# Dyllon-Preston/trajopt-grpo

Hardware: AMD Instinct MI355X
Metric: env-steps/sec at 65k parallel quadrotor envs (rollout + PPO update) (higher is better)
Workload: dtype bf16 (f32 accumulate) MLP; f32 env / returns / loss / optimizer

## Files before the change

### include/trajopt_grpo_hip.h

```cpp
#ifndef TRAJOPT_GRPO_HIP_H
#define TRAJOPT_GRPO_HIP_H

#include <stdint.h>

#ifdef __cplusplus
extern "C" {
#endif

#define TG_ABI_VERSION 13

enum { TG_OK = 0, TG_ERR_ARG = -1, TG_ERR_HIP = -2, TG_ERR_UNSUPPORTED = -3 };

#define TG_ACT_RELU 0
#define TG_ACT_TANH 1

enum { TG_ENV_CARTPOLE = 0, TG_ENV_QUADPOLE2D = 1, TG_ENV_QUADPOLE = 2, TG_ENV_QUADROTOR12 = 3, TG_ENV_PENDULUM = 4 };
enum { TG_F32 = 0, TG_F64 = 1 };

typedef struct tg_env_params {
    int32_t env_id;
    int32_t max_steps;
    int32_t time_trunc_step;
    int32_t agents;
    double  timestep;
    double  p[12];
} tg_env_params;

typedef struct tg_traj {
    void*     d_obs;
    float*    d_act;
    void*     d_rew;
    uint8_t*  d_mask;
    int32_t*  d_len;
    uint64_t* d_counters;
    int64_t   n;
    int32_t   horizon;
    int32_t   dtype;
} tg_traj;

const char* tg_last_error(void);
int  tg_abi_version(void);
int  tg_chain_depth_kernels(int on);

int  tg_env_dims(int env_id, int* obs_dim, int* act_dim);
int  tg_env_default_params(int env_id, int max_steps, tg_env_params* out);
int  tg_env_finalize_params(tg_env_params* p);

int  tg_env_reset(const tg_env_params* p, int dtype, void* d_state, int64_t ld, int64_t n,
                  uint64_t seed, uint64_t stream_id, int64_t key_offset, int64_t key_div,
                  void* stream);

int  tg_env_step(const tg_env_params* p, int dtype, const void* d_state, int64_t ld,
                 const float* d_action, int64_t ld_a, void* d_next, int64_t ld_next,
                 int32_t* d_steps, void* d_time_balanced, void* d_reward,
                 uint8_t* d_truncated, int64_t n, void* stream);

int  tg_quadrotor12_dynamics(const tg_env_params* p, int dtype, const void* d_state, int64_t ld,
                             const void* d_control, int64_t ld_c, void* d_next, int64_t ld_next,
                             int64_t n, void* stream);


int  tg_rollout_begin(const tg_traj* tr, int obs_dim, int act_dim, void* stream);

int  tg_rollout_step(const tg_env_params* p, const tg_traj* tr, int32_t t, const float* d_mean,
                     int64_t mean_row_stride, const float* sigma, const uint64_t* d_rng,
// ... 499 lines not shown
```

### trajopt-grpo_amd/_native.py

```python
from __future__ import annotations

import ctypes as C
import os

import torch

_HERE = os.path.dirname(os.path.abspath(__file__))
LIB_PATH = os.environ.get("TG_NATIVE_LIB") or os.path.join(_HERE, "libtrajopt_grpo_hip.so")
ABI_VERSION = 13

TG_ENV_CARTPOLE, TG_ENV_QUADPOLE2D, TG_ENV_QUADPOLE, TG_ENV_QUADROTOR12, TG_ENV_PENDULUM = 0, 1, 2, 3, 4
TG_F32, TG_F64 = 0, 1
TG_OK, TG_ERR_ARG, TG_ERR_HIP, TG_ERR_UNSUPPORTED = 0, -1, -2, -3
TG_ACT_RELU, TG_ACT_TANH = 0, 1
ENV_IDS = {"CartPole": TG_ENV_CARTPOLE, "QuadPole2D": TG_ENV_QUADPOLE2D, "QuadPole": TG_ENV_QUADPOLE,
           "Quadrotor": TG_ENV_QUADROTOR12, "Pendulum": TG_ENV_PENDULUM}


class NativeLibraryError(RuntimeError):
    pass


class EnvParams(C.Structure):
    _fields_ = [("env_id", C.c_int32), ("max_steps", C.c_int32), ("time_trunc_step", C.c_int32),
# ... 92 lines not shown
                ("d_act_rows", C.c_void_p), ("d_idx", C.c_void_p), ("d_src0", C.c_void_p), ("d_dst0", C.c_void_p),
                ("d_src1", C.c_void_p), ("d_dst1", C.c_void_p), ("d_moments", C.c_void_p), ("group_size", C.c_int64),
                ("rows_cap", C.c_int64)]


class VecEnv(C.Structure):
    _fields_ = [("d_state", C.c_void_p), ("d_steps", C.c_void_p), ("d_balanced", C.c_void_p), ("d_ep_return", C.c_void_p),
                ("d_episode", C.c_void_p), ("n", C.c_int64), ("env_offset", C.c_int64), ("seed", C.c_uint64), ("horizon", C.c_int32),
                ("dtype", C.c_int32)]


class Replay(C.Structure):
    _fields_ = [("d_obs", C.c_void_p), ("d_act", C.c_void_p), ("d_next_obs", C.c_void_p), ("d_rew", C.c_void_p), ("d_disc", C.c_void_p),
                ("d_nstep", C.c_void_p), ("d_last_obs", C.c_void_p), ("d_cursor", C.c_void_p), ("d_filled", C.c_void_p),
                ("d_open", C.c_void_p), ("n", C.c_int64), ("capacity_steps", C.c_int32), ("obs_dim", C.c_int32), ("act_dim", C.c_int32),
                ("n_step", C.c_int32), ("discount", C.c_float * 17)]


_P, _I32, _I64, _U64, _F, _VP = C.POINTER, C.c_int32, C.c_int64, C.c_uint64, C.c_float, C.c_void_p
SIGNATURES = {
    "tg_last_error": (C.c_char_p, []),
    "tg_abi_version": (C.c_int, []),
    "tg_chain_depth_kernels": (C.c_int, [C.c_int]),
    "tg_env_dims": (C.c_int, [C.c_int, _P(C.c_int), _P(C.c_int)]),
    "tg_env_default_params": (C.c_int, [C.c_int, C.c_int, _P(EnvParams)]),
    "tg_env_finalize_params": (C.c_int, [_P(EnvParams)]),
    "tg_env_reset": (C.c_int, [_P(EnvParams), C.c_int, _VP, _I64, _I64, _U64, _U64, _I64, _I64, _VP]),
    "tg_env_step": (C.c_int, [_P(EnvParams), C.c_int, _VP, _I64, _VP, _I64, _VP, _I64, _VP, _VP, _VP, _VP, _I64, _VP]),
    "tg_quadrotor12_dynamics": (C.c_int, [_P(EnvParams), C.c_int, _VP, _I64, _VP, _I64, _VP, _I64, _I64, _VP]),
    "tg_rollout_begin": (C.c_int, [_P(Traj), C.c_int, C.c_int, _VP]),
    "tg_rollout_step": (C.c_int, [_P(EnvParams), _P(Traj), _I32, _VP, _I64, _P(_F), _VP, _I64, _VP]),
    "tg_rollout_forced": (C.c_int, [_P(EnvParams), _P(Traj), _I32, _I32, _VP]),
    "tg_rollout_final_state": (C.c_int, [_P(EnvParams), _P(Traj), _VP, _VP, _VP]),
    "tg_rollout_finish": (C.c_int, [_P(Traj), _VP]),
    "tg_rollout_finish_stats_workspace": (C.c_int, []),
    "tg_rollout_finish_stats": (C.c_int, [_P(Traj), _VP, _VP, _VP, _VP]),
    "tg_fused_rollout": (C.c_int, [_P(EnvParams), _P(Traj), _VP, _VP, _I32, _I32, _P(_F), _VP, _I64, _I32, _I32, _VP]),
    "tg_fused_rollout_f32_supported": (C.c_int, [_I32, _I32]),
    "tg_fused_rollout_f32_block_envs": (C.c_int, [_I64, _I32]),
    "tg_fused_rollout_f32": (C.c_int, [_P(EnvParams), _P(Traj), _VP, _VP, _I32, _I32, _I32, _P(_F), _VP, _I64, _I32, _I32, _VP]),
    "tg_fused_rollout_f32_act": (C.c_int, [_P(EnvParams), _P(Traj), _VP, _VP, _I32, _I32, _I32, _P(_F), _VP, _I64, _I32, _I32, _I32, _VP]),
    "tg_rng_advance": (C.c_int, [_VP, _VP]),
    "tg_env_randomize": (C.c_int, [_P(EnvParams), _P(RandomizeSpec), _VP, _I64, _U64, _U64, _I64, _I64, _VP]),
    "tg_rollout_step_dr": (C.c_int, [_P(EnvParams), _VP, _P(Traj), _I32, _VP, _I64, _P(_F), _VP, _I64, _VP]),
    "tg_rollout_forced_dr": (C.c_int, [_P(EnvParams), _VP, _P(Traj), _I32, _I32, _VP]),
    "tg_rollout_final_state_dr": (C.c_int, [_P(EnvParams), _VP, _P(Traj), _VP, _VP, _VP]),
# ... 193 lines not shown
        raise RuntimeError(f"{what or 'trajopt_grpo_hip'} failed ({rc}): {msg}")


def require_cuda(*tensors):
    for t in tensors:
        if t is not None and not t.is_cuda:
            raise NativeLibraryError("the HIP rollout path needs tensors on an MI355X (cuda) device; got a CPU tensor. "
                                     "There is no CPU fallback.")


def ptr(t):
    return 0 if t is None else t.data_ptr()


RAW_PARAM_WRITES = [0]
ALWAYS_REBUILD = os.environ.get("TG_ALWAYS_REBUILD", "0") == "1"
TRUST_KEYS = os.environ.get("TG_TRUST_VERSION_KEYS", "0") == "1"


def chain_depth_kernels_default():
    return os.environ.get("TG_CHAIN_DEPTH_KERNELS", "1") != "0"


def event_pair():
    return (torch.cuda.Event(enable_timing=True), torch.cuda.Event(enable_timing=True))


def stream_ptr(device=None):
    return torch.cuda.current_stream(device).cuda_stream


def dtype_code(dt):
    if dt == torch.float32:
        return TG_F32
    if dt == torch.float64:
        return TG_F64
    raise ValueError(f"state dtype must be float32 or float64, got {dt}")


def default_params(env_id, max_steps):
    p = EnvParams()
    check(load().tg_env_default_params(env_id, int(max_steps), C.byref(p)), "tg_env_default_params")
    return p


def env_dims(env_id):
# ... 4 lines not shown
```

### trajopt-grpo_amd/csrc/api_common.cpp

```cpp
#include "tg_common.hpp"
#include <atomic>

namespace tg {

static thread_local char g_err[512] = "";

int set_error(int code, const char* fmt, ...) {
    va_list ap;
    va_start(ap, fmt);
    vsnprintf(g_err, sizeof(g_err), fmt, ap);
    va_end(ap);
    return code;
}

static std::atomic<int> g_chain_depth_kernels{1};
bool chain_depth_kernels() { return g_chain_depth_kernels.load(std::memory_order_relaxed) != 0; }

}

extern "C" {
const char* tg_last_error(void) { return tg::g_err; }
int tg_abi_version(void) { return TG_ABI_VERSION; }
int tg_chain_depth_kernels(int on) { return tg::g_chain_depth_kernels.exchange(on != 0 ? 1 : 0, std::memory_order_relaxed); }

int tg_clock_probe_attach(int32_t family, void* d_probe) {
    switch (family) {
        case TG_PROBE_FWD_CHAIN: return tg::attach_probe_fwd_chain(d_probe);
        case TG_PROBE_BWD_CHAIN: return tg::attach_probe_bwd_chain(d_probe);
        case TG_PROBE_WEIGHT_GRAD: return tg::attach_probe_weight_grad(d_probe);
        case TG_PROBE_F32_CHAIN: { const int rc = tg::attach_probe_f32(0, d_probe); return rc ? rc : tg::attach_probe_f32w(0, d_probe); }
        case TG_PROBE_F32_WEIGHT_GRAD: { const int rc = tg::attach_probe_f32(1, d_probe); return rc ? rc : tg::attach_probe_f32w(1, d_probe); }
        case TG_PROBE_MFMA_LOOP: return tg::attach_probe_mfma_loop(d_probe);
        case TG_PROBE_FWD_CHAIN_PLAIN: return tg::attach_probe_fwd_chain_plain(d_probe);
        default: return tg::set_error(TG_ERR_ARG, "tg_clock_probe_attach: family %d", family);
    }
}
}
```

### trajopt-grpo_amd/csrc/mfma_ring.hpp

```cpp
#pragma once
#include "tg_common.hpp"

namespace tg {

typedef __bf16 bf16x8 __attribute__((ext_vector_type(8)));
typedef float f32x16 __attribute__((ext_vector_type(16)));
typedef float f32x4 __attribute__((ext_vector_type(4)));
typedef __attribute__((address_space(3))) void lds_void;

typedef unsigned int act_u32x4 __attribute__((ext_vector_type(4)));
__device__ static inline void act_store16(act_u32x4 v, act_u32x4* p) {
    __builtin_nontemporal_store(v, p);
}

template <int H>
struct PanelOrder {
    static constexpr int CG = H / 32;
    static constexpr int ROWQ = CG * 256;
    static constexpr int PANEL = 8 * ROWQ;
    __host__ __device__ static constexpr int64_t chunk_off(int64_t row, int c) {
        return (row >> 5) * PANEL + ((row >> 2) & 7) * ROWQ + (c >> 2) * 256 + (row & 3) * 64 + (c & 3) * 16;
    }
    __host__ __device__ static constexpr int64_t store_row(int64_t row, int64_t rows) {
        return row < ((rows + 31) & ~(int64_t)31) ? row : rows - 1;
// ... 56 lines not shown
    CUR = ring + cur_slot * KS * 64;                                                                       \
    cur_slot = (cur_slot + 1 == D) ? 0 : cur_slot + 1;
#define TG_RING_NEXT    \
    const uint4* cur;   \
    TG_RING_NEXT_INTO(cur)
#define TG_RING_ADVANCE(WAITN) TG_RING_WAIT(WAITN) TG_RING_NEXT

template <int KS, int WPW, int D, int NB>
__device__ static inline const uint4* ring_next_at(const uint4*& wfrag, uint4* ring, int c, int wave, uint32_t& voff) {
    static_assert(NB % D == 0, "the ring must be back at slot 0 after every round");
    constexpr int P = D - 1;
    __builtin_amdgcn_s_barrier();
    asm volatile("" : "+v"(voff), "+s"(wfrag) : : "memory");
    const char* gblock = reinterpret_cast<const char*>(wfrag) + ((c + P) % NB) * (KS * 1024);
    uint4* slot = ring + ((c + P) % D) * (KS * 64);
#pragma unroll
    for (int q = 0; q < KS / WPW; ++q) {
        const int piece = q * WPW + wave;
        __builtin_amdgcn_global_load_lds(reinterpret_cast<const uint4*>(gblock + piece * 1024 + voff), (lds_void*)(slot + piece * 64), 16, 0, 0);
    }
    return ring + (c % D) * (KS * 64);
}

}
```

### trajopt-grpo_amd/csrc/mlp_fwd_chain.hip

```cpp
#include "mfma_ring.hpp"
#include "loss_row.hpp"

namespace tg {

typedef float f32x4 __attribute__((ext_vector_type(4)));

constexpr int kChainMaxHidden = 8;
TG_CLOCK_PROBE_VAR(g_probe_fwd_chain, attach_probe_fwd_chain)
TG_CLOCK_PROBE_VAR(g_probe_fwd_chain_plain, attach_probe_fwd_chain_plain)
struct ChainActs { uint16_t* p[kChainMaxHidden]; uint32_t* m[kChainMaxHidden]; };

struct ChainLoss {
    int32_t kind, A;
    const float* act;
    const float* logp_old; const float* adv;
    float n_m, n_i;
    float inv_var[4]; float logp_const, epsilon, surr_coef, critic_coef, kl_coef;
    const float* norm8;
    uint16_t* dout8;
    float* head_slabs;
    double* work;
    float* bias_partial;
    const float* logp_ref; float ref_coef;
    const float* log_std; float* std_out;
// ... 74 lines not shown
    f32x4 acc[2][2];
#pragma unroll
    for (int f = 0; f < 2; ++f) {
        const float4 b4 = lds_float4(b8 + 4 * f);
#pragma unroll
        for (int c = 0; c < 2; ++c) acc[f][c] = f32x4{b4.x, b4.y, b4.z, b4.w};
    }
    __builtin_amdgcn_s_setprio(1);
#pragma unroll
    for (int ks = 0; ks < K8; ++ks)
#pragma unroll
        for (int f = 0; f < 2; ++f) {
            const bf16x8 a = __builtin_bit_cast(bf16x8, cur[(ks * 2 + f) * 64 + lane]);
#pragma unroll
            for (int c = 0; c < 2; ++c) acc[f][c] = __builtin_amdgcn_mfma_f32_16x16x32_bf16(a, xin[c][ks], acc[f][c], 0, 0, 0);
        }
    __builtin_amdgcn_s_setprio(0);
#pragma unroll
    for (int c = 0; c < 2; ++c)
        out[c] = relu_pack_bf16(acc[0][c][0], acc[0][c][1], acc[0][c][2], acc[0][c][3], acc[1][c][0], acc[1][c][1], acc[1][c][2],
                                acc[1][c][3]);
}

__device__ static inline int wave_of(unsigned tid) { return (int)(tid >> 6); }

#define TG_CHAIN_ADVANCE(WAITN) TG_RING_ADVANCE(WAITN)

template <int H, int WPW, bool kStore, int D, bool kA0, bool kHead = false, bool kRef = false, bool kStd = false, bool kPanel = false>
__global__ __launch_bounds__(64 * WPW, 2) void mlp_fwd_chain_kernel(const uint16_t* __restrict__ x, const uint4* __restrict__ wfrag,
                                                                    const float* __restrict__ bias, int32_t n_hh, int64_t rows,
                                                                    ChainActs acts, float* __restrict__ out, int32_t out_cols,
                                                                    ChainLoss L) {
    static_assert(!kHead || (kStore && !kA0), "the fused head belongs to the learner's training pass");
    static_assert(!kRef || kHead, "the reference penalty is a term of the fused head");
    static_assert(!kStd || kHead, "the learned log-std is a term of the fused head");
    static_assert(!kPanel || (kStore && D == 4), "panel order is a layout of the stored activations; its wait counts are for P = 3");
    if constexpr (kHead) loss_from_device<kStd>(L);
    constexpr int MT = H / 32, KS = H / 16, K8 = H / 32;
    constexpr int P = D - 1;
    static_assert(P % 2 == 1 && P >= 3, "the store counts below are for a window of an odd number of blocks");
    constexpr int kWaitEven = (P - 1) * (KS / WPW) + (kStore ? 4 * ((P + 1) / 2) : 0);
    constexpr int kWaitOdd = (P - 1) * (KS / WPW) + (kStore ? 4 * ((P - 1) / 2) : 0);
    constexpr int kWaitMin = (P - 1) * (KS / WPW);
#define TG_PANEL_WAIT(S)                                                                    \
    if ((S) == 0) { TG_RING_WAIT(kWaitMin) } else if ((S) == 1) { TG_RING_WAIT(kWaitMin + 2) } \
    else if ((S) == 2) { TG_RING_WAIT(kWaitMin + 4) } else { TG_RING_WAIT(kWaitMin + 6) }
    static_assert(KS % WPW == 0, "every wave moves the same number of 1-KiB pieces per block");
    extern __shared__ uint4 lds[];
    uint4* ring = lds;
    float* bias_s = reinterpret_cast<float*>(lds + D * KS * 64);
    uint4* xs = reinterpret_cast<uint4*>(bias_s + (n_hh + 2) * H);
    uint4* stage = xs + WPW * 128 + wave_of(threadIdx.x) * (32 * 8);
#define TG_HEAD_LDS                                                                                                              \
    char* tiles = reinterpret_cast<char*>(xs + WPW * 128);                                                                       \
    char* dtiles = tiles + WPW * 32 * 128;                                                                                       \
    [[maybe_unused]] float* lin = reinterpret_cast<float*>(dtiles + WPW * 1024) + wave_of(threadIdx.x) * 256;                    \
    [[maybe_unused]] double* sums_d = reinterpret_cast<double*>(dtiles + 2 * WPW * 1024) + (wave_of(threadIdx.x) * 16 + (threadIdx.x & 15)) * 4; \
    [[maybe_unused]] float* sums_f = reinterpret_cast<float*>(dtiles + 2 * WPW * 1024 + WPW * 16 * 32) + (wave_of(threadIdx.x) * 16 + (threadIdx.x & 15)) * 4; \
    [[maybe_unused]] float* hacc = reinterpret_cast<float*>(dtiles + 2 * WPW * 1024 + WPW * 16 * 48) + (wave_of(threadIdx.x) * MT * 16 + (threadIdx.x & 15)) * 4;

    const int lane = threadIdx.x & 63, wave = threadIdx.x >> 6;
    const int grp = lane >> 4, col = lane & 15;
    const int64_t n_rounds = (rows + 32 * WPW - 1) / (32 * WPW);
    const int n_blocks = n_hh * MT + 2;
    if constexpr (kHead) { TG_CLOCK_PROBE_BEGIN(g_probe_fwd_chain) } else { TG_CLOCK_PROBE_BEGIN(g_probe_fwd_chain_plain) }

    for (int q = threadIdx.x; q < (n_hh + 2) * H; q += 64 * WPW) bias_s[q] = bias[q];
    if constexpr (kHead) {
        TG_HEAD_LDS
        if (grp == 0) {
#pragma unroll
            for (int b = 0; b < MT; ++b) *reinterpret_cast<float4*>(hacc + b * 64) = float4{0.f, 0.f, 0.f, 0.f};
            lds_stored2(sums_d, double2{0.0, 0.0});
            lds_stored2(sums_d + 2, double2{0.0, 0.0});
            *reinterpret_cast<float4*>(sums_f) = float4{0.f, 0.f, 0.f, 0.f};
        }
    }
    __syncthreads();

    uint4* my_xs = xs + wave * 128;
    auto dma_x = [&](int64_t round) {
        const int64_t base = round * (32 * WPW) + wave * 32;
#pragma unroll
        for (int p = 0; p < 2; ++p) {
// ... 10 lines not shown
            int64_t r = round * (32 * WPW) + wave * 32 + lane;
            r = r < rows ? r : rows - 1;
            if (L.kind != 1) {
#pragma unroll
                for (int k = 0; k < 4; ++k)
                    if (k < L.A) __builtin_amdgcn_global_load_lds(L.act + r * L.A + k, (lds_void*)(lin + 32 * k), 4, 0, 0);
                __builtin_amdgcn_global_load_lds(L.logp_old + r, (lds_void*)(lin + 32 * 4), 4, 0, 0);
                __builtin_amdgcn_global_load_lds(L.adv + r, (lds_void*)(lin + 32 * 5), 4, 0, 0);
                if constexpr (kRef) __builtin_amdgcn_global_load_lds(L.logp_ref + r, (lds_void*)(lin + 32 * 6), 4, 0, 0);
            } else {
                __builtin_amdgcn_global_load_lds(L.act + r, (lds_void*)(lin + 32 * 0), 4, 0, 0);
            }
        }
    };
    int pre_pos = 0, pre_slot = 0, cur_slot = 0;
    dma_x(blockIdx.x);
    if constexpr (kHead) dma_loss_inputs(blockIdx.x);
    for (int b0 = 0; b0 < P; ++b0) {
        ring_dma_block<KS, WPW>(wfrag + (int64_t)pre_pos * KS * 64, ring + pre_slot * KS * 64, wave, lane);
        pre_pos = (pre_pos + 1 == n_blocks) ? 0 : pre_pos + 1;
        pre_slot = (pre_slot + 1 == D) ? 0 : pre_slot + 1;
    }
    asm volatile("s_waitcnt vmcnt(0)" ::: "memory");

    for (int64_t round = blockIdx.x; round < n_rounds; round += gridDim.x) {
        const int64_t row0 = round * (32 * WPW) + wave * 32;
        int64_t rowc[2];
#pragma unroll
        for (int c = 0; c < 2; ++c) {
            rowc[c] = row0 + 16 * c + col;
            rowc[c] = rowc[c] < rows ? rowc[c] : rows - 1;
        }
        bf16x8 xin[2][K8], xout[2][K8];
        [[maybe_unused]] int64_t poff[2];
        if constexpr (kPanel) {
#pragma unroll
            for (int c = 0; c < 2; ++c) poff[c] = PanelOrder<H>::chunk_off(PanelOrder<H>::store_row(row0 + 16 * c + col, rows), grp);
        }

        {
            if constexpr (kHead) { TG_RING_WAIT(kWaitMin) } else { TG_RING_WAIT(kWaitOdd) }
            TG_RING_NEXT
            bf16x8 x0[2];
#pragma unroll
            for (int c = 0; c < 2; ++c) x0[c] = __builtin_bit_cast(bf16x8, lds_read_b128_opaque(my_xs + (16 * c + col) * 4 + grp));
            dma_x(round + gridDim.x);
#pragma unroll
            for (int mt = 0; mt < MT; ++mt) {
                f32x4 acc[2][2];
#pragma unroll
                for (int f = 0; f < 2; ++f) {
                    const float4 b4 = lds_float4(bias_s + 32 * mt + 8 * grp + 4 * f);
                    const bf16x8 a = __builtin_bit_cast(bf16x8, cur[(mt * 2 + f) * 64 + lane]);
#pragma unroll
                    for (int c = 0; c < 2; ++c)
                        acc[f][c] = __builtin_amdgcn_mfma_f32_16x16x32_bf16(a, x0[c], f32x4{b4.x, b4.y, b4.z, b4.w}, 0, 0, 0);
                }
#pragma unroll
                for (int c = 0; c < 2; ++c)
                    xout[c][mt] = relu_pack_bf16(acc[0][c][0], acc[0][c][1], acc[0][c][2], acc[0][c][3], acc[1][c][0], acc[1][c][1],
                                                 acc[1][c][2], acc[1][c][3]);
                if constexpr (kPanel) {
                    if (kA0) {
                        const bf16x8 pv[2] = {xout[0][mt], xout[1][mt]};
                        store_panel<H>(acts.p[0], poff, mt, pv);
                    }
                } else if (kStore && kA0 && (mt & 1)) {
                    const bf16x8 pa[2] = {xout[0][mt - 1], xout[1][mt - 1]}, pb[2] = {xout[0][mt], xout[1][mt]};
                    store_pair(stage, acts.p[0] + 32 * (mt - 1), row0, rows, H, lane, pa, pb);
                }
            }
#pragma unroll
            for (int c = 0; c < 2; ++c)
#pragma unroll
                for (int ks = 0; ks < K8; ++ks) xin[c][ks] = xout[c][ks];
        }
        for (int l = 0; l < n_hh; ++l) {
            const float* bl = bias_s + (l + 1) * H + 8 * grp;
            uint32_t mw[2][MT / 2];
#pragma unroll
            for (int mt = 0; mt < MT; ++mt) {
                const bool top_layer = kHead && l == n_hh - 1;
                if constexpr (kPanel) {
                    const int same = mt < 3 ? mt : 3;
                    if (top_layer) { TG_PANEL_WAIT(3 - same) } else if (l == 0) { TG_PANEL_WAIT(same) } else { TG_PANEL_WAIT(3) }
                } else if ((kStore && !kA0 && l == 0 && mt < 3) || (top_layer && mt >= 3)) {
                    TG_RING_WAIT(kWaitMin)
                } else if ((mt & 1) || (top_layer && mt == 2)) {
                    TG_RING_WAIT(kWaitOdd)
                } else {
                    TG_RING_WAIT(kWaitEven)
                }
                TG_RING_NEXT
                if (kStore) {
                    const int q = mt;
                    mw[q / (MT / 2)][q % (MT / 2)] = pair_mask_word(xin[q / (MT / 2)], q % (MT / 2), 4 * (grp & 1));
                }
                bf16x8 o[2];
                chain_block<K8>(cur, bl + 32 * mt, xin, o, lane);
                xout[0][mt] = o[0];
                xout[1][mt] = o[1];
                if constexpr (kPanel) {
                    if (mt == MT - 1 && acts.m[l]) {
#pragma unroll
                        for (int c = 0; c < 2; ++c) store_mask_words<MT>(acts.m[l], rowc[c], grp, mw[c]);
                    }
                    if (!top_layer) store_panel<H>(acts.p[l + 1], poff, mt, o);
                } else if (mt & 1) {
                    if (kStore && mt == MT - 1 && acts.m[l]) {
#pragma unroll
                        for (int c = 0; c < 2; ++c) store_mask_words<MT>(acts.m[l], rowc[c], grp, mw[c]);
                    }
                    if (kStore && !top_layer) {
                        const bf16x8 pa[2] = {xout[0][mt - 1], xout[1][mt - 1]}, pb[2] = {xout[0][mt], xout[1][mt]};
                        store_pair(stage, acts.p[l + 1] + 32 * (mt - 1), row0, rows, H, lane, pa, pb);
                    }
                }
            }
#pragma unroll
            for (int c = 0; c < 2; ++c)
#pragma unroll
                for (int ks = 0; ks < K8; ++ks) xin[c][ks] = xout[c][ks];
        }
        {
            if constexpr (kHead) { TG_RING_WAIT(kWaitMin) } else if constexpr (kPanel) { TG_PANEL_WAIT(3) } else { TG_RING_WAIT(kWaitEven) }
            TG_RING_NEXT
            if (kStore && acts.m[n_hh]) {
#pragma unroll
                for (int c = 0; c < 2; ++c) {
                    uint32_t mw[MT / 2];
#pragma unroll
                    for (int i = 0; i < MT / 2; ++i) mw[i] = pair_mask_word(xin[c], i, 4 * (grp & 1));
                    store_mask_words<MT>(acts.m[n_hh], rowc[c], grp, mw);
                }
            }
            const float4 b4 = lds_float4(bias_s + (n_hh + 1) * H + 4 * grp);
            f32x4 acc[2] = {f32x4{b4.x, b4.y, b4.z, b4.w}, f32x4{b4.x, b4.y, b4.z, b4.w}};
#pragma unroll
            for (int ks = 0; ks < K8; ++ks) {
                const bf16x8 a = __builtin_bit_cast(bf16x8, cur[(ks * 2) * 64 + lane]);
#pragma unroll
                for (int c = 0; c < 2; ++c) acc[c] = __builtin_amdgcn_mfma_f32_16x16x32_bf16(a, xin[c][ks], acc[c], 0, 0, 0);
            }
            if (out != nullptr && 4 * grp < out_cols) {
#pragma unroll
                for (int c = 0; c < 2; ++c)
                    *reinterpret_cast<float4*>(out + rowc[c] * out_cols + 4 * grp) = float4{acc[c][0], acc[c][1], acc[c][2], acc[c][3]};
            }
            if constexpr (kHead) {
                TG_HEAD_LDS
                char* dt = dtiles + wave * 1024;
                if (grp == 0) {
#pragma unroll 1
                    for (int c = 0; c < 2; ++c) {
                        float c_surr = 0.f, c_crit = 0.f, c_kl = 0.f, c_cnt = 0.f;
                        const int rl = 16 * c + col;
                        const bool valid = row0 + rl < rows;
                        float g[4] = {0.f, 0.f, 0.f, 0.f};
                        const f32x4 mu = c == 0 ? acc[0] : acc[1];
                        const int64_t rc = c == 0 ? rowc[0] : rowc[1];
                        if (valid) {
                            if (L.kind != 1) {
                                const Gauss4 G = loss_gauss4(L);
// ... 59 lines not shown
                    asm volatile("s_waitcnt lgkmcnt(0)" ::: "memory");
                    __builtin_amdgcn_s_barrier();
                    asm volatile("" ::: "memory");
                    if (b + 1 < MT) write_tile(b + 1);
                    f32x4 t = {};
#pragma unroll
                    for (int ks = 0; ks < 2; ++ks) {
                        const int v = 2 * (wave >> 1) + ks;
                        const char* db = dtiles + v * 1024;
                        const char* tb = tiles + ((b & 1) * WPW + v) * 2048;
                        const bf16x8 fa = tr_frag16(db + d_lo, db + d_hi), fb = tr_frag16(tb + t_lo, tb + t_hi);
                        t = __builtin_amdgcn_mfma_f32_16x16x32_bf16(fa, fb, t, 0, 0, 0);
                    }
                    if (grp == 0) {
                        const float4 h = lds_float4(hacc + b * 64);
                        lds_store16(reinterpret_cast<char*>(hacc + b * 64),
                                    __builtin_bit_cast(uint4, float4{h.x + t[0], h.y + t[1], h.z + t[2], h.w + t[3]}));
                    }
                }
                asm volatile("s_waitcnt lgkmcnt(0)" ::: "memory");
                dma_loss_inputs(round + gridDim.x);
            }
        }
    }
    if constexpr (kHead) {
        TG_HEAD_LDS
        float* slab = L.head_slabs + ((int64_t)blockIdx.x * 4 + (wave >> 1)) * 16 * H;
        if (grp == 0) {
#pragma unroll
            for (int b = 0; b < MT; ++b) {
                const float4 h = lds_float4(hacc + b * 64);
                const float hv[4] = {h.x, h.y, h.z, h.w};
#pragma unroll
                for (int r = 0; r < 4; ++r) slab[r * H + 32 * b + 16 * (wave & 1) + col] = hv[r];
            }
        }
        __syncthreads();
        if (threadIdx.x < 8) {
            const int j = threadIdx.x & 3;
            if (threadIdx.x < 4) {
                double t = 0.0;
                const double* sd = reinterpret_cast<const double*>(dtiles + 2 * WPW * 1024);
                for (int q = 0; q < WPW * 16; ++q) t += sd[q * 4 + j];
                L.work[(int64_t)blockIdx.x * 4 + j] = t;
            } else {
                float t = 0.f;
                const float* sf = reinterpret_cast<const float*>(dtiles + 2 * WPW * 1024 + WPW * 16 * 32);
                for (int q = 0; q < WPW * 16; ++q) t += sf[q * 4 + j];
                L.bias_partial[(int64_t)blockIdx.x * 4 + j] = t;
            }
        }
    }
    asm volatile("s_waitcnt vmcnt(0)" ::: "memory");
    if constexpr (kHead) { TG_CLOCK_PROBE_END(g_probe_fwd_chain) } else { TG_CLOCK_PROBE_END(g_probe_fwd_chain_plain) }
}

template <int H, bool kStore, int D, bool kA0, bool kHead = false, bool kRef = false, bool kStd = false, bool kPanel = false>
static int chain_launch(const void* x, const void* wfrag, const float* bias, int n_hh, int64_t rows, const ChainActs& acts, float* out,
                        int out_cols, hipStream_t st, const ChainLoss& loss = ChainLoss{}) {
    constexpr int WPW = 8, KS = H / 16;
    const size_t shmem = (size_t)D * KS * 1024 + (size_t)(n_hh + 2) * H * sizeof(float) + (size_t)WPW * 2048 +
                         (kPanel && !kHead ? 0 : (size_t)WPW * 32 * 128) + (kHead ? (size_t)2 * WPW * 1024 + (size_t)WPW * 16 * 48 + (size_t)WPW * (H / 32) * 16 * 16 : 0);
    auto kern = mlp_fwd_chain_kernel<H, WPW, kStore, D, kA0, kHead, kRef, kStd, kPanel>;
    static LdsOptIn opt_in;
    if (int rc = reserve_dynamic_lds((const void*)kern, shmem, opt_in, "tg_mlp_forward_chain")) return rc;
    const int cus = device_cus();
    const int64_t n_rounds = ceil_div(rows, (int64_t)32 * WPW);
    const unsigned grid = (unsigned)(n_rounds < cus ? n_rounds : cus);
    hipLaunchKernelGGL(kern, dim3(grid), dim3(64 * WPW), shmem, st, (const uint16_t*)x, (const uint4*)wfrag, bias, n_hh, rows, acts, out,
                       out_cols, loss);
    TG_LAUNCH_CHECK("tg_mlp_forward_chain");
    return TG_OK;
}

}

using namespace tg;

extern "C" {

static int forward_chain(const void* d_x, const void* d_wfrag, const float* d_bias, int32_t hidden, int32_t n_hidden_layers,
                         int64_t rows, void* const* d_acts, void* const* d_masks, float* d_out, int32_t out_cols, int32_t layout,
                         void* stream) {
    TG_REQUIRE(d_x && d_wfrag && d_bias && d_out, "tg_mlp_forward_chain: null pointer");
    TG_REQUIRE(hidden == 128 || hidden == 256, "tg_mlp_forward_chain: hidden width %d unsupported (128, 256)", hidden);
    TG_REQUIRE(n_hidden_layers >= 1 && n_hidden_layers <= kChainMaxHidden, "tg_mlp_forward_chain: %d hidden layers outside 1..%d",
// ... 63 lines not shown
               "tg_mlp_forward_chain_loss: missing per-row input");
    TG_REQUIRE(loss->kind == 1 || (loss->act_col_stride == 1 && loss->act_row_stride == loss->act_dim),
               "tg_mlp_forward_chain_loss: the actions must be contiguous [rows][act_dim]");

    TG_REQUIRE(rows > 0, "tg_mlp_forward_chain_loss: no rows");
    ChainActs acts{};
    for (int l = 0; l < n_hidden_layers; ++l) {
        TG_REQUIRE(d_masks[l] && (d_acts[l] || l == 0 || l == n_hidden_layers - 1), "tg_mlp_forward_chain_loss: buffer %d is null", l);
        acts.p[l] = (uint16_t*)d_acts[l];
        acts.m[l] = (uint32_t*)d_masks[l];
    }
    TG_REQUIRE(!d_acts[0], "tg_mlp_forward_chain_loss: the first activation is recomputed by tg_mlp_weight_grad, not stored");
    ChainLoss L{};
    fill_loss_common(L, loss, use_ref ? ref : nullptr, use_std ? std : nullptr);
    if (loss->kind == 0 && loss->d_logp_old_out != nullptr) {
        L.kind = 2;
        L.logp_old = loss->d_logp_old_out;
    }
    L.dout8 = (uint16_t*)loss->d_dout8; L.head_slabs = loss->d_head_slabs; L.work = loss->d_work; L.bias_partial = loss->d_bias_partial;
    hipStream_t st = (hipStream_t)stream;
    const int n_hh = n_hidden_layers - 1;
    if (layout == TG_LAYOUT_PANEL) {
        TG_REQUIRE(!use_std && !use_ref, "tg_mlp_forward_chain_loss_ex: panel order is built for the plain head only");
        return hidden == 256 ? chain_launch<256, true, 4, false, true, false, false, true>(d_x, d_wfrag, d_bias, n_hh, rows, acts, nullptr, 8, st, L)
                             : chain_launch<128, true, 4, false, true, false, false, true>(d_x, d_wfrag, d_bias, n_hh, rows, acts, nullptr, 8, st, L);
    }
    if (use_std) {
        if (use_ref)
            return hidden == 256 ? chain_launch<256, true, 4, false, true, true, true>(d_x, d_wfrag, d_bias, n_hh, rows, acts, nullptr, 8, st, L)
                                 : chain_launch<128, true, 4, false, true, true, true>(d_x, d_wfrag, d_bias, n_hh, rows, acts, nullptr, 8, st, L);
        return hidden == 256 ? chain_launch<256, true, 4, false, true, false, true>(d_x, d_wfrag, d_bias, n_hh, rows, acts, nullptr, 8, st, L)
                             : chain_launch<128, true, 4, false, true, false, true>(d_x, d_wfrag, d_bias, n_hh, rows, acts, nullptr, 8, st, L);
    }
    if (use_ref)
        return hidden == 256 ? chain_launch<256, true, 4, false, true, true>(d_x, d_wfrag, d_bias, n_hh, rows, acts, nullptr, 8, st, L)
                             : chain_launch<128, true, 4, false, true, true>(d_x, d_wfrag, d_bias, n_hh, rows, acts, nullptr, 8, st, L);
    return hidden == 256 ? chain_launch<256, true, 4, false, true>(d_x, d_wfrag, d_bias, n_hh, rows, acts, nullptr, 8, st, L)
                         : chain_launch<128, true, 4, false, true>(d_x, d_wfrag, d_bias, n_hh, rows, acts, nullptr, 8, st, L);
}

int tg_mlp_forward_chain_loss(const void* d_x, const void* d_wfrag, const float* d_bias, int32_t hidden, int32_t n_hidden_layers,
                              int64_t rows, void* const* d_acts, void* const* d_masks, const tg_chain_loss* loss, void* stream) {
    return forward_chain_loss(d_x, d_wfrag, d_bias, hidden, n_hidden_layers, rows, d_acts, d_masks, loss, nullptr, stream);
}

int tg_mlp_forward_chain_loss_ref(const void* d_x, const void* d_wfrag, const float* d_bias, int32_t hidden, int32_t n_hidden_layers,
// ... 19 lines not shown
```

### trajopt-grpo_amd/csrc/tg_common.hpp

```cpp
#pragma once
#include <hip/hip_runtime.h>
#include <stdint.h>
#include <stdarg.h>
#include <stdio.h>

#include "../../include/trajopt_grpo_hip.h"

namespace tg {

int set_error(int code, const char* fmt, ...);
bool chain_depth_kernels();

#define TG_REQUIRE(cond, ...)                                   \
    do {                                                        \
        if (!(cond)) return ::tg::set_error(TG_ERR_ARG, __VA_ARGS__); \
    } while (0)

#define TG_LAUNCH_CHECK(what)                                                        \
    do {                                                                             \
        hipError_t e__ = hipGetLastError();                                          \
        if (e__ != hipSuccess)                                                       \
            return ::tg::set_error(TG_ERR_HIP, "%s: %s", what, hipGetErrorString(e__)); \
    } while (0)

constexpr int kWave = 64;

__device__ static inline float rn_mul(float a, float b) {
#pragma clang fp contract(off)
    return a * b;
}
__device__ static inline float rn_add(float a, float b) {
#pragma clang fp contract(off)
    return a + b;
}
// ... 168 lines not shown
```

### trajopt-grpo_amd/mlp.py

```python
from __future__ import annotations

import ctypes as C
import logging

import torch

from . import _native as N
from . import hip_ops as K

_ROW_BLOCK = 8192


_LOG = logging.getLogger("trajopt_grpo_amd")
_LOGGED_SHAPES = set()

def _mark_ones_column(xp: torch.Tensor) -> None:
    lo = xp.storage_offset() * xp.element_size()
    xp.untyped_storage()._tg_ones = (lo, lo + xp.numel() * xp.element_size(), xp.shape[1] * xp.element_size())


def set_ones_column(xp: torch.Tensor, has: bool) -> None:
    if has:
        _mark_ones_column(xp)
    elif getattr(xp.untyped_storage(), "_tg_ones", None) is not None:
# ... 176 lines not shown
            self._buf[name] = b = torch.empty(max(rows, cap_rows, self.default_cap) * cols, dtype=dtype, device=device)
        return b[:need].view(rows, cols)


class GemmMLP:
    def __init__(self, net, compute_dtype=torch.bfloat16):
        self.act = hidden_activation(net)
        if self.act == "Tanh":
            if compute_dtype != torch.float32 or not f32_chain_supported(net):
                raise ValueError("GemmMLP runs a Tanh net only in float32 on the fp32 chain learner (Linear(S<=32, H) Tanh "
                                 "[Linear(H, H) Tanh]{0..3} Linear(H, A<=4), H in {64, 128})")
        else:
            assert supports(net, compute_dtype)
        self.net = net
        self.cd = compute_dtype
        self.linears = [m for m in net.network if isinstance(m, torch.nn.Linear)]
        dev = self.linears[0].weight.device
        self.in_dim, self.out_dim = self.linears[0].in_features, self.linears[-1].out_features
        self._f32 = None
        self.f32_store_all = False
        self.panel_order = True
        self.panel_mixed = False
        self.depth_kernels = N.chain_depth_kernels_default()
        if self.act == "Tanh":
            self._f32 = F32ChainStream(net, f32_chain_supported(net), activation="Tanh")
            self.f32_store_all = True
        elif compute_dtype == torch.float32 and f32_res_supported(net):
            self._f32 = F32ResStream(net)
        elif compute_dtype == torch.float32 and f32_chain_supported(net):
            self._f32 = F32ChainStream(net, f32_chain_supported(net))
        elif compute_dtype == torch.float32 and f32_wide_supported(net):
            self._f32 = F32WideStream(net)
        self.in_pad = _round_up(self.in_dim, 32) if self._f32 is None else self._f32.in_pad
        self.out_pad = _round_up(self.out_dim, 8)
        self.w, self.b = [], []
        for i, l in enumerate(self.linears):
            o = self.out_pad if i == len(self.linears) - 1 else l.out_features
            k = self.in_pad if i == 0 else l.in_features
            self.w.append(torch.zeros(o, k, dtype=compute_dtype, device=dev))
            self.b.append(torch.zeros(o, dtype=compute_dtype, device=dev))
        self._acts = None
        self._bits = None
        self._ws = _Workspace()
        self._partial = None
        self._dxfrag = [None] * len(self.linears)
        if compute_dtype == torch.bfloat16:
# ... 203 lines not shown
        assert self.act == "ReLU"
        self._flush_riders()
        self._fresh("chain")
        L = len(self.linears)
        rows, H, dev = xp.shape[0], self._chain.H, xp.device
        panel = bool(self.panel_order) and PANEL_ORDER_HEAD_PASS and ref is None and std is None
        hid = [None if i in (0, L - 2) else self._ws.get(f"a{i}", _round_up(rows, 32) if panel else rows, H, self.cd, dev)
               for i in range(L - 1)]
        bits = [self._ws.get(f"m{i}", rows, H // 32, torch.int32, dev) for i in range(L - 1)]
        dz_head = self._ws.get("z_head", rows, self.out_pad, self.cd, dev)
        nblk = lib.tg_mlp_forward_chain_blocks()
        if self._head_ws is None:
            self._head_ws = (torch.empty(nblk * 4 * 16 * H, dtype=torch.float32, device=dev),
                             torch.empty(nblk * 4, dtype=torch.float64, device=dev),
                             torch.empty(nblk * 4, dtype=torch.float32, device=dev))
        slabs, work, bpart = self._head_ws
        a = self._loss_args(kind, rows, act, logp_old, adv, ret, norm, var, epsilon, surr_coef, critic_coef, kl_coef, logp_old_out, norm8)
        a.d_dout8, a.d_head_slabs, a.d_work, a.d_bias_partial = dz_head.data_ptr(), slabs.data_ptr(), work.data_ptr(), bpart.data_ptr()
        ptrs = (N.C.c_void_p * (L - 1))(*[N.ptr(t) or None for t in hid])
        mptrs = (N.C.c_void_p * (L - 1))(*[t.data_ptr() for t in bits])
        name, tail, targs = loss_entry("bf16", N.TG_ACT_RELU, ref, std)
        if panel:
            name, tail, targs = "tg_mlp_forward_chain_loss_ex", (None, None, N.TG_LAYOUT_PANEL), ",false,false,true"
        ev = None
        if self.fwd_events is not None:
            ev = N.event_pair()
            ev[0].record()
        N.check(getattr(lib, name)(xp.data_ptr(), self._chain.stream.data_ptr(), self._chain.bias.data_ptr(), H, L - 1, rows, ptrs, mptrs,
                                   N.C.byref(a), *tail, N.stream_ptr(dev)), name)
        self._acts_panel = panel
        if ev is not None:
            ev[1].record()
            stored = sum(1 for t in hid if t is not None)
            per_row = (2 * self.in_pad + stored * 2 * H + (L - 1) * (H // 8) + 16 + (4 * self.out_dim + 8 if kind == 0 else 4) + (4 if ref else 0)
                       + (16 if std else 0))
            self.fwd_events.append((ev[0], ev[1], rows, per_row, f"tg::mlp_fwd_chain_kernel<{H},8,true,4,false,true{targs}>"))
        grid = min(nblk, -(-rows // 256))
        lin = self.linears[-1]
        self._riders = ([(slabs, 0, 16 * H, grid * 4, H, lin.weight.grad, self.out_dim, H),
                         (bpart, 0, 4, grid, 4, lin.bias.grad, 1, self.out_dim)],
                        (work, grid, sums_out) if sums_out is not None else None)
        if sums_out is not None:
            assert sums_out.dtype == torch.float64 and sums_out.is_cuda and sums_out.numel() == 4 and sums_out.is_contiguous()
        self._acts = [xp] + hid
        self._bits = [None] + bits
        self._dz_head = dz_head
        return None if sums_out is not None else work[:grid * 4].view(grid, 4).sum(0)

    def _set_depth_kernels(self, lib):
        on = bool(self.depth_kernels)
        lib.tg_chain_depth_kernels(int(on))
        return on

    def _flush_riders(self):
        riders, loss_rider = getattr(self, "_riders", None) or ([], None)
        self._riders = None
        for slab, off, stride, n_slabs, pitch, grad, m_out, n_out in riders:
            if n_slabs > 0:
                v = torch.as_strided(slab, (n_slabs, m_out, n_out), (stride, pitch, 1), off).sum(0)
                grad.add_(v.view_as(grad))
        if loss_rider is not None:
            work, n, sums = loss_rider
            sums += work[:n * 4].view(n, 4).sum(0)

    def _loss_args(self, kind, rows, act, logp_old, adv, ret, norm, var, epsilon, surr_coef, critic_coef, kl_coef, logp_old_out=None,
                   norm8=None) -> "N.ChainLoss":
        a = N.ChainLoss()
        if norm8 is not None:
            N.require_cuda(norm8)
            assert norm8.dtype == torch.float32 and norm8.is_contiguous() and norm8.numel() == 8
            a.d_norm8 = norm8.data_ptr()
        a.kind, a.act_dim = kind, self.out_dim
        if kind == 0:
            N.require_cuda(act, logp_old, adv, logp_old_out)
# ... 687 lines not shown
```

Measured before the change: 8.611 million.

## Add block-structured hidden-layer pass to panel forward-chain kernel for H=256

Adds a kBlk variant of the fused forward-chain-with-loss kernel for H=256 in panel layout, enabled by default through a new runtime toggle. Each hidden layer is processed one 32-row block at a time. Per block, the next weight block is prefetched with global_load_lds into a wave-relative LDS ring, fragment pairs are read with inline-asm ds_read_b128 under raised wave priority, and activations go out as nontemporal stores with 32-bit offsets. The aim is to overlap weight streaming with MFMA work and cut address arithmetic in the layer loop, at the cost of hand-tuned wait counts and an H=256-only code path.

```diff
diff --git a/include/trajopt_grpo_hip.h b/include/trajopt_grpo_hip.h
--- a/include/trajopt_grpo_hip.h
+++ b/include/trajopt_grpo_hip.h
@@ -41,6 +41,7 @@
 const char* tg_last_error(void);
 int  tg_abi_version(void);
 int  tg_chain_depth_kernels(int on);
+int  tg_chain_fwd_kernels(int on);
 
 int  tg_env_dims(int env_id, int* obs_dim, int* act_dim);
 int  tg_env_default_params(int env_id, int max_steps, tg_env_params* out);
diff --git a/trajopt-grpo_amd/_native.py b/trajopt-grpo_amd/_native.py
--- a/trajopt-grpo_amd/_native.py
+++ b/trajopt-grpo_amd/_native.py
@@ -138,6 +138,7 @@
     "tg_last_error": (C.c_char_p, []),
     "tg_abi_version": (C.c_int, []),
     "tg_chain_depth_kernels": (C.c_int, [C.c_int]),
+    "tg_chain_fwd_kernels": (C.c_int, [C.c_int]),
     "tg_env_dims": (C.c_int, [C.c_int, _P(C.c_int), _P(C.c_int)]),
     "tg_env_default_params": (C.c_int, [C.c_int, C.c_int, _P(EnvParams)]),
     "tg_env_finalize_params": (C.c_int, [_P(EnvParams)]),
@@ -377,6 +378,10 @@
     return os.environ.get("TG_CHAIN_DEPTH_KERNELS", "1") != "0"
 
 
+def chain_fwd_kernels_default():
+    return os.environ.get("TG_CHAIN_FWD_KERNELS", "1") != "0"
+
+
 def event_pair():
     return (torch.cuda.Event(enable_timing=True), torch.cuda.Event(enable_timing=True))
 
diff --git a/trajopt-grpo_amd/csrc/api_common.cpp b/trajopt-grpo_amd/csrc/api_common.cpp
--- a/trajopt-grpo_amd/csrc/api_common.cpp
+++ b/trajopt-grpo_amd/csrc/api_common.cpp
@@ -15,6 +15,8 @@
 
 static std::atomic<int> g_chain_depth_kernels{1};
 bool chain_depth_kernels() { return g_chain_depth_kernels.load(std::memory_order_relaxed) != 0; }
+static std::atomic<int> g_chain_fwd_kernels{1};
+bool chain_fwd_kernels() { return g_chain_fwd_kernels.load(std::memory_order_relaxed) != 0; }
 
 }
 
@@ -22,6 +24,7 @@
 const char* tg_last_error(void) { return tg::g_err; }
 int tg_abi_version(void) { return TG_ABI_VERSION; }
 int tg_chain_depth_kernels(int on) { return tg::g_chain_depth_kernels.exchange(on != 0 ? 1 : 0, std::memory_order_relaxed); }
+int tg_chain_fwd_kernels(int on) { return tg::g_chain_fwd_kernels.exchange(on != 0 ? 1 : 0, std::memory_order_relaxed); }
 
 int tg_clock_probe_attach(int32_t family, void* d_probe) {
     switch (family) {
diff --git a/trajopt-grpo_amd/csrc/mfma_ring.hpp b/trajopt-grpo_amd/csrc/mfma_ring.hpp
--- a/trajopt-grpo_amd/csrc/mfma_ring.hpp
+++ b/trajopt-grpo_amd/csrc/mfma_ring.hpp
@@ -102,4 +102,20 @@
     return ring + (c % D) * (KS * 64);
 }
 
+template <int KS, int WPW>
+__device__ static inline const uint4* ring_next_rel(const char*& src, int off, const uint4* const (&rd)[2], const uint32_t (&m0b)[2], int j,
+                                                    uint32_t& voff) {
+    __builtin_amdgcn_s_barrier();
+    asm volatile("" : "+v"(voff), "+s"(src) : : "memory");
+    const int jd = (j + 3) & 3;
+    const uint32_t dst = m0b[jd >> 1] + (jd & 1) * (KS * 1024);
+#pragma unroll
+    for (int q = 0; q < KS / WPW; ++q) {
+        const char* piece = src + off + q * (WPW * 1024);
+        asm volatile("" : "+s"(piece));
+        __builtin_amdgcn_global_load_lds(reinterpret_cast<const uint4*>(piece + voff), (lds_void*)(uintptr_t)(dst + q * (WPW * 1024)), 16, 0, 0);
+    }
+    return rd[(j & 3) >> 1] + (j & 1) * (KS * 64);
 }
+
+}
diff --git a/trajopt-grpo_amd/csrc/mlp_fwd_chain.hip b/trajopt-grpo_amd/csrc/mlp_fwd_chain.hip
--- a/trajopt-grpo_amd/csrc/mlp_fwd_chain.hip
+++ b/trajopt-grpo_amd/csrc/mlp_fwd_chain.hip
@@ -120,11 +120,46 @@
                                 acc[1][c][3]);
 }
 
+#define TG_FRAG_PAIR(A0, A1, BASE, OFF)                                                                              \
+    asm volatile("ds_read_b128 %0, %2 offset:" #OFF "\n\tds_read_b128 %1, %2 offset:" #OFF "+1024\n\ts_waitcnt lgkmcnt(0)" \
+                 : "=&v"(A0), "=&v"(A1)                                                                               \
+                 : "v"(BASE)                                                                                         \
+                 : "memory");
+#define TG_PAIR_KSTEP(KS)                                                                                            \
+    {                                                                                                                \
+        uint4 a0, a1;                                                                                                \
+        if (second) { TG_FRAG_PAIR(a0, a1, base, 16384+KS*2048) } else { TG_FRAG_PAIR(a0, a1, base, KS*2048) }       \
+        _Pragma("unroll") for (int c = 0; c < 2; ++c)                                                                \
+            acc[0][c] = __builtin_amdgcn_mfma_f32_16x16x32_bf16(__builtin_bit_cast(bf16x8, a0), xin[c][KS], acc[0][c], 0, 0, 0); \
+        _Pragma("unroll") for (int c = 0; c < 2; ++c)                                                                \
+            acc[1][c] = __builtin_amdgcn_mfma_f32_16x16x32_bf16(__builtin_bit_cast(bf16x8, a1), xin[c][KS], acc[1][c], 0, 0, 0); \
+    }
+__device__ static inline void chain_block_pairs(uint32_t base, bool second, const float* __restrict__ b8, const bf16x8 (&xin)[2][8],
+                                                bf16x8 (&out)[2]) {
+    f32x4 acc[2][2];
+#pragma unroll
+    for (int f = 0; f < 2; ++f) {
+        const float4 b4 = lds_float4(b8 + 4 * f);
+#pragma unroll
+        for (int c = 0; c < 2; ++c) acc[f][c] = f32x4{b4.x, b4.y, b4.z, b4.w};
+    }
+    __builtin_amdgcn_s_setprio(1);
+    TG_PAIR_KSTEP(0) TG_PAIR_KSTEP(1) TG_PAIR_KSTEP(2) TG_PAIR_KSTEP(3) TG_PAIR_KSTEP(4) TG_PAIR_KSTEP(5) TG_PAIR_KSTEP(6) TG_PAIR_KSTEP(7)
+    __builtin_amdgcn_s_setprio(0);
+#pragma unroll
+    for (int c = 0; c < 2; ++c)
+        out[c] = relu_pack_bf16(acc[0][c][0], acc[0][c][1], acc[0][c][2], acc[0][c][3], acc[1][c][0], acc[1][c][1], acc[1][c][2],
+                                acc[1][c][3]);
+}
+#undef TG_PAIR_KSTEP
+#undef TG_FRAG_PAIR
+
 __device__ static inline int wave_of(unsigned tid) { return (int)(tid >> 6); }
 
 #define TG_CHAIN_ADVANCE(WAITN) TG_RING_ADVANCE(WAITN)
 
-template <int H, int WPW, bool kStore, int D, bool kA0, bool kHead = false, bool kRef = false, bool kStd = false, bool kPanel = false>
+template <int H, int WPW, bool kStore, int D, bool kA0, bool kHead = false, bool kRef = false, bool kStd = false, bool kPanel = false,
+          bool kBlk = false>
 __global__ __launch_bounds__(64 * WPW, 2) void mlp_fwd_chain_kernel(const uint16_t* __restrict__ x, const uint4* __restrict__ wfrag,
                                                                     const float* __restrict__ bias, int32_t n_hh, int64_t rows,
                                                                     ChainActs acts, float* __restrict__ out, int32_t out_cols,
@@ -133,6 +168,7 @@
     static_assert(!kRef || kHead, "the reference penalty is a term of the fused head");
     static_assert(!kStd || kHead, "the learned log-std is a term of the fused head");
     static_assert(!kPanel || (kStore && D == 4), "panel order is a layout of the stored activations; its wait counts are for P = 3");
+    static_assert(!kBlk || (H == 256 && WPW == 8 && kHead && kPanel && !kRef && !kStd), "the block-structured pass is the learner's plain head");
     if constexpr (kHead) loss_from_device<kStd>(L);
     constexpr int MT = H / 32, KS = H / 16, K8 = H / 32;
     constexpr int P = D - 1;
@@ -157,7 +193,8 @@
     [[maybe_unused]] float* sums_f = reinterpret_cast<float*>(dtiles + 2 * WPW * 1024 + WPW * 16 * 32) + (wave_of(threadIdx.x) * 16 + (threadIdx.x & 15)) * 4; \
     [[maybe_unused]] float* hacc = reinterpret_cast<float*>(dtiles + 2 * WPW * 1024 + WPW * 16 * 48) + (wave_of(threadIdx.x) * MT * 16 + (threadIdx.x & 15)) * 4;
 
-    const int lane = threadIdx.x & 63, wave = threadIdx.x >> 6;
+    const int lane = threadIdx.x & 63;
+    const int wave = kBlk ? __builtin_amdgcn_readfirstlane(threadIdx.x >> 6) : (int)(threadIdx.x >> 6);
     const int grp = lane >> 4, col = lane & 15;
     const int64_t n_rounds = (rows + 32 * WPW - 1) / (32 * WPW);
     const int n_blocks = n_hh * MT + 2;
@@ -214,6 +251,19 @@
         pre_slot = (pre_slot + 1 == D) ? 0 : pre_slot + 1;
     }
     asm volatile("s_waitcnt vmcnt(0)" ::: "memory");
+    [[maybe_unused]] const uint4* rd[2] = {ring + lane, ring + 2 * KS * 64 + lane};
+    [[maybe_unused]] uint32_t m0b[2] = {(uint32_t)(uintptr_t)(__attribute__((address_space(3))) uint4*)ring + 1024u * (uint32_t)wave, 0u};
+    m0b[1] = m0b[0] + 2u * KS * 1024u;
+    [[maybe_unused]] const char* wsrc = reinterpret_cast<const char*>(wfrag);
+    [[maybe_unused]] uint32_t voff = 16u * threadIdx.x;
+    const int rl = kBlk ? 0 : lane;
+#define TG_FWD_RING_NEXT(J, POS)                                                          \
+    const uint4* cur;                                                                     \
+    if constexpr (kBlk) {                                                                 \
+        cur = ring_next_rel<KS, WPW>(wsrc, (POS) * (KS * 1024), rd, m0b, (J), voff);      \
+    } else {                                                                              \
+        TG_RING_NEXT_INTO(cur)                                                            \
+    }
 
     for (int64_t round = blockIdx.x; round < n_rounds; round += gridDim.x) {
         const int64_t row0 = round * (32 * WPW) + wave * 32;
@@ -229,10 +279,16 @@
 #pragma unroll
             for (int c = 0; c < 2; ++c) poff[c] = PanelOrder<H>::chunk_off(PanelOrder<H>::store_row(row0 + 16 * c + col, rows), grp);
         }
+        [[maybe_unused]] const int64_t round_off = round * (WPW * (int64_t)PanelOrder<H>::PANEL);
+        [[maybe_unused]] uint32_t poff32[2];
+        if constexpr (kBlk) {
+#pragma unroll
+            for (int c = 0; c < 2; ++c) poff32[c] = (uint32_t)(poff[c] - round_off);
+        }
 
         {
             if constexpr (kHead) { TG_RING_WAIT(kWaitMin) } else { TG_RING_WAIT(kWaitOdd) }
-            TG_RING_NEXT
+            TG_FWD_RING_NEXT(0, 3)
             bf16x8 x0[2];
 #pragma unroll
             for (int c = 0; c < 2; ++c) x0[c] = __builtin_bit_cast(bf16x8, lds_read_b128_opaque(my_xs + (16 * c + col) * 4 + grp));
@@ -243,7 +299,7 @@
 #pragma unroll
                 for (int f = 0; f < 2; ++f) {
                     const float4 b4 = lds_float4(bias_s + 32 * mt + 8 * grp + 4 * f);
-                    const bf16x8 a = __builtin_bit_cast(bf16x8, cur[(mt * 2 + f) * 64 + lane]);
+                    const bf16x8 a = __builtin_bit_cast(bf16x8, cur[(mt * 2 + f) * 64 + rl]);
 #pragma unroll
                     for (int c = 0; c < 2; ++c)
                         acc[f][c] = __builtin_amdgcn_mfma_f32_16x16x32_bf16(a, x0[c], f32x4{b4.x, b4.y, b4.z, b4.w}, 0, 0, 0);
@@ -267,7 +323,7 @@
 #pragma unroll
                 for (int ks = 0; ks < K8; ++ks) xin[c][ks] = xout[c][ks];
         }
-        for (int l = 0; l < n_hh; ++l) {
+        for (int l = 0; l < (kBlk ? 0 : n_hh); ++l) {
             const float* bl = bias_s + (l + 1) * H + 8 * grp;
             uint32_t mw[2][MT / 2];
 #pragma unroll
@@ -314,9 +370,27 @@
 #pragma unroll
                 for (int ks = 0; ks < K8; ++ks) xin[c][ks] = xout[c][ks];
         }
+        if constexpr (kBlk) {
+            const char* lay = wsrc + KS * 1024;
+            {
+                constexpr bool kFirst = true, kTop = false;
+                constexpr int l = 0;
+#include "mlp_fwd_chain_layer.inc"
+            }
+#pragma unroll 1
+            for (int l = 1; l < n_hh - 1; ++l) {
+                constexpr bool kFirst = false, kTop = false;
+#include "mlp_fwd_chain_layer.inc"
+            }
+            {
+                constexpr bool kFirst = false, kTop = true;
+                const int l = n_hh - 1;
+#include "mlp_fwd_chain_layer.inc"
+            }
+        }
         {
             if constexpr (kHead) { TG_RING_WAIT(kWaitMin) } else if constexpr (kPanel) { TG_PANEL_WAIT(3) } else { TG_RING_WAIT(kWaitEven) }
-            TG_RING_NEXT
+            TG_FWD_RING_NEXT(1, 2)
             if (kStore && acts.m[n_hh]) {
 #pragma unroll
                 for (int c = 0; c < 2; ++c) {
@@ -330,7 +404,7 @@
             f32x4 acc[2] = {f32x4{b4.x, b4.y, b4.z, b4.w}, f32x4{b4.x, b4.y, b4.z, b4.w}};
 #pragma unroll
             for (int ks = 0; ks < K8; ++ks) {
-                const bf16x8 a = __builtin_bit_cast(bf16x8, cur[(ks * 2) * 64 + lane]);
+                const bf16x8 a = __builtin_bit_cast(bf16x8, cur[(ks * 2) * 64 + rl]);
 #pragma unroll
                 for (int c = 0; c < 2; ++c) acc[c] = __builtin_amdgcn_mfma_f32_16x16x32_bf16(a, xin[c][ks], acc[c], 0, 0, 0);
             }
@@ -436,7 +510,16 @@
                 dma_loss_inputs(round + gridDim.x);
             }
         }
-    }
+        if constexpr (kBlk) {
+            const uint4* r0 = rd[0];
+            rd[0] = rd[1];
+            rd[1] = r0;
+            const uint32_t m0 = m0b[0];
+            m0b[0] = m0b[1];
+            m0b[1] = m0;
+        }
+    }
+#undef TG_FWD_RING_NEXT
     if constexpr (kHead) {
         TG_HEAD_LDS
         float* slab = L.head_slabs + ((int64_t)blockIdx.x * 4 + (wave >> 1)) * 16 * H;
@@ -469,13 +552,14 @@
     if constexpr (kHead) { TG_CLOCK_PROBE_END(g_probe_fwd_chain) } else { TG_CLOCK_PROBE_END(g_probe_fwd_chain_plain) }
 }
 
-template <int H, bool kStore, int D, bool kA0, bool kHead = false, bool kRef = false, bool kStd = false, bool kPanel = false>
+template <int H, bool kStore, int D, bool kA0, bool kHead = false, bool kRef = false, bool kStd = false, bool kPanel = false,
+          bool kBlk = false>
 static int chain_launch(const void* x, const void* wfrag, const float* bias, int n_hh, int64_t rows, const ChainActs& acts, float* out,
                         int out_cols, hipStream_t st, const ChainLoss& loss = ChainLoss{}) {
     constexpr int WPW = 8, KS = H / 16;
     const size_t shmem = (size_t)D * KS * 1024 + (size_t)(n_hh + 2) * H * sizeof(float) + (size_t)WPW * 2048 +
                          (kPanel && !kHead ? 0 : (size_t)WPW * 32 * 128) + (kHead ? (size_t)2 * WPW * 1024 + (size_t)WPW * 16 * 48 + (size_t)WPW * (H / 32) * 16 * 16 : 0);
-    auto kern = mlp_fwd_chain_kernel<H, WPW, kStore, D, kA0, kHead, kRef, kStd, kPanel>;
+    auto kern = mlp_fwd_chain_kernel<H, WPW, kStore, D, kA0, kHead, kRef, kStd, kPanel, kBlk>;
     static LdsOptIn opt_in;
     if (int rc = reserve_dynamic_lds((const void*)kern, shmem, opt_in, "tg_mlp_forward_chain")) return rc;
     const int cus = device_cus();
@@ -585,6 +669,8 @@
     const int n_hh = n_hidden_layers - 1;
     if (layout == TG_LAYOUT_PANEL) {
         TG_REQUIRE(!use_std && !use_ref, "tg_mlp_forward_chain_loss_ex: panel order is built for the plain head only");
+        if (hidden == 256 && chain_fwd_kernels())
+            return chain_launch<256, true, 4, false, true, false, false, true, true>(d_x, d_wfrag, d_bias, n_hh, rows, acts, nullptr, 8, st, L);
         return hidden == 256 ? chain_launch<256, true, 4, false, true, false, false, true>(d_x, d_wfrag, d_bias, n_hh, rows, acts, nullptr, 8, st, L)
                              : chain_launch<128, true, 4, false, true, false, false, true>(d_x, d_wfrag, d_bias, n_hh, rows, acts, nullptr, 8, st, L);
     }
diff --git a/trajopt-grpo_amd/csrc/mlp_fwd_chain_layer.inc b/trajopt-grpo_amd/csrc/mlp_fwd_chain_layer.inc
--- /dev/null
+++ b/trajopt-grpo_amd/csrc/mlp_fwd_chain_layer.inc
@@ -0,0 +1,42 @@
+            {
+                const float* bl = bias_s + (l + 1) * H + 8 * grp;
+                typedef __attribute__((address_space(1))) char global_char;
+                global_char* pl = kTop ? nullptr : (global_char*)(reinterpret_cast<char*>(acts.p[l + 1]) + round_off);
+                typedef __attribute__((address_space(1))) uint32_t global_u32;
+                global_u32* mlg = (global_u32*)acts.m[l];
+                asm volatile("" : "+s"(pl), "+s"(mlg));
+                uint32_t* ml = (uint32_t*)mlg;
+                uint32_t mw[2][MT / 2];
+#pragma unroll
+                for (int mt = 0; mt < MT; ++mt) {
+                    const int same = mt < 3 ? mt : 3;
+                    __builtin_amdgcn_sched_barrier(0);
+                    if (kTop) { TG_PANEL_WAIT(3 - same) } else if (kFirst) { TG_PANEL_WAIT(same) } else { TG_PANEL_WAIT(3) }
+                    if (kTop && mt + 3 >= MT + 1) ring_next_rel<KS, WPW>(wsrc, (mt + 3 - (MT + 1)) * (KS * 1024), rd, m0b, 1 + mt, voff);
+                    else ring_next_rel<KS, WPW>(lay, (mt + 3) * (KS * 1024), rd, m0b, 1 + mt, voff);
+                    mw[mt / (MT / 2)][mt % (MT / 2)] = pair_mask_word(xin[mt / (MT / 2)], mt % (MT / 2), 4 * (grp & 1));
+                    bf16x8 o[2];
+                    chain_block_pairs((uint32_t)(uintptr_t)(__attribute__((address_space(3))) const uint4*)rd[((1 + mt) & 3) >> 1], (1 + mt) & 1,
+                                      bl + 32 * mt, xin, o);
+                    xout[0][mt] = o[0];
+                    xout[1][mt] = o[1];
+                    if (mt == MT - 1) {
+#pragma unroll
+                        for (int c = 0; c < 2; ++c) store_mask_words<MT>(ml, rowc[c], grp, mw[c]);
+                    }
+                    if (!kTop) {
+#pragma unroll
+                        for (int c = 0; c < 2; ++c) {
+                            const uint4 u = __builtin_bit_cast(uint4, o[c]);
+                            asm volatile("" : "+v"(poff32[c]));
+                            __builtin_nontemporal_store(act_u32x4{u.x, u.y, u.z, u.w},
+                                                        (__attribute__((address_space(1))) act_u32x4*)(pl + poff32[c] + mt * 256));
+                        }
+                    }
+                }
+#pragma unroll
+                for (int c = 0; c < 2; ++c)
+#pragma unroll
+                    for (int ks = 0; ks < K8; ++ks) xin[c][ks] = xout[c][ks];
+                lay += MT * (KS * 1024);
+            }
diff --git a/trajopt-grpo_amd/csrc/tg_common.hpp b/trajopt-grpo_amd/csrc/tg_common.hpp
--- a/trajopt-grpo_amd/csrc/tg_common.hpp
+++ b/trajopt-grpo_amd/csrc/tg_common.hpp
@@ -10,6 +10,7 @@
 
 int set_error(int code, const char* fmt, ...);
 bool chain_depth_kernels();
+bool chain_fwd_kernels();
 
 #define TG_REQUIRE(cond, ...)                                   \
     do {                                                        \
diff --git a/trajopt-grpo_amd/mlp.py b/trajopt-grpo_amd/mlp.py
--- a/trajopt-grpo_amd/mlp.py
+++ b/trajopt-grpo_amd/mlp.py
@@ -222,6 +222,7 @@
         self.panel_order = True
         self.panel_mixed = False
         self.depth_kernels = N.chain_depth_kernels_default()
+        self.fwd_depth_kernels = N.chain_fwd_kernels_default()
         if self.act == "Tanh":
             self._f32 = F32ChainStream(net, f32_chain_supported(net), activation="Tanh")
             self.f32_store_all = True
@@ -471,6 +472,8 @@
         name, tail, targs = loss_entry("bf16", N.TG_ACT_RELU, ref, std)
         if panel:
             name, tail, targs = "tg_mlp_forward_chain_loss_ex", (None, None, N.TG_LAYOUT_PANEL), ",false,false,true"
+            if self._set_fwd_depth_kernels(lib) and H == 256:
+                targs += ",true"
         ev = None
         if self.fwd_events is not None:
             ev = N.event_pair()
@@ -499,6 +502,11 @@
     def _set_depth_kernels(self, lib):
         on = bool(self.depth_kernels)
         lib.tg_chain_depth_kernels(int(on))
+        return on
+
+    def _set_fwd_depth_kernels(self, lib):
+        on = bool(self.fwd_depth_kernels)
+        lib.tg_chain_fwd_kernels(int(on))
         return on
 
     def _flush_riders(self):
```

Result: faster. 8.773 million, median of 6 (+1.9%).
